# viniciusvidal2/slam-sensor-fusion

Measured on AMD Instinct MI355X. Metric: scans_per_s_200k_scan_vs_10M_map, higher is better.
Workload: dtype f32 points / f64 accumulation

## Files before the change

### include/slamfusion.h

```cpp
#ifndef SLAMFUSION_H
#define SLAMFUSION_H
#include <stdint.h>

#ifdef __cplusplus
extern "C" {
#endif

#define SF_VERSION 210

typedef enum {
    SF_OK = 0,
    SF_ERR_INVALID = -1,
    SF_ERR_HIP = -2,
    SF_ERR_NOMEM = -3,
    SF_ERR_STATE = -4,
    SF_ERR_OVERFLOW = -5,
    SF_ERR_COMM = -6
} sf_status;

typedef struct sf_ctx sf_ctx;
typedef struct sf_cloud sf_cloud;
typedef struct sf_map sf_map;
typedef struct sf_icp sf_icp;

// ... 126 lines not shown
int sf_icp_fused_count(sf_icp *icp, int64_t *launches);
int sf_icp_fused_redone(sf_icp *icp, int64_t *redone);
int sf_icp_test_inject_barrier_timeout(sf_icp *icp);
#define SF_ORDER_AUTO 0
#define SF_ORDER_AS_GIVEN 1
#define SF_ORDER_CELL 2
int sf_icp_set_query_order(sf_icp *icp, int order);
int sf_icp_set_nn_reuse(sf_icp *icp, int on);
int sf_icp_set_wide_scan_points(sf_icp *icp, int64_t points);
int sf_icp_set_pipeline(sf_icp *icp, int on);
int sf_icp_set_tile_search(sf_icp *icp, int mode);
int sf_icp_tile_info(sf_icp *icp, int64_t out[12]);
int sf_icp_set_freeze(sf_icp *icp, int on);
int sf_icp_set_freeze_params(sf_icp *icp, float guard_scale, float guard_min, float guard_max, int max_tries, int from_launch);
int sf_icp_freeze_stats(sf_icp *icp, int64_t out[5]);
#define SF_ROBUST_NONE 0
#define SF_ROBUST_HUBER 1
#define SF_ROBUST_CAUCHY 2
#define SF_ROBUST_TUKEY 3
#define SF_ROBUST_GM 4
int sf_icp_set_robust_kernel(sf_icp *icp, int kind, double k);

#define SF_COV_EIG_EPS 1e-12
#define SF_COV_FEW_CORR 1
#define SF_COV_SINGULAR 2
#define SF_COV_DEGENERATE_TRANS 4
#define SF_COV_DEGENERATE_ROT 8
typedef struct {
    double info[36];
    double cov[36];
// ... 188 lines not shown
```

### slam_sensor_fusion_amd/api.py

```python
import atexit
import ctypes as C
import os
import weakref

import numpy as np

_HERE = os.path.dirname(os.path.abspath(__file__))
LIB_PATH = os.path.join(_HERE, "lib", "libslamfusion.so")

SF_ICP_REF_CPP, SF_ICP_O3D_P2P, SF_ICP_P2PLANE = 0, 1, 2
SF_VOXEL_PCL, SF_VOXEL_O3D, SF_VOXEL_PCL64 = 0, 1, 2
SF_FLAG_VOXEL_OVERFLOW = 1
SF_ICP_FLAG_FEW_CORR, SF_ICP_FLAG_SINGULAR, SF_ICP_FLAG_SHARD_STALE, SF_ICP_FLAG_BARRIER_TIMEOUT = 1, 2, 4, 8
PROF_NN, PROF_REDUCE, PROF_COLLECTIVE, PROF_SOLVE, PROF_SHARD_BUILD = 0, 1, 2, 3, 4
SF_ERR_COMM = -6
MODES = {"ref_cpp": SF_ICP_REF_CPP, "o3d_p2p": SF_ICP_O3D_P2P, "p2plane": SF_ICP_P2PLANE}
ROBUST_KINDS = {"none": 0, "huber": 1, "cauchy": 2, "tukey": 3, "gm": 4}


class SlamFusionError(RuntimeError):
    pass


class IcpResult(C.Structure):
# ... 556 lines not shown

    def tile_info(self):
        a = (C.c_int64 * 12)()
        _check(self.lib.sf_icp_tile_info(self.h, a))
        return {"on": bool(a[0]), "cells_per_tile": [a[1], a[2], a[3]], "tiles": [a[4], a[5], a[6]], "searched": a[7], "from_lds": a[8], "left_region": a[9],
                "beyond_ring_1": a[10], "tiles_too_dense": a[11]}

    def set_freeze_params(self, guard_scale=8.0, guard_min=2.0e-5, guard_max=3.0e-4, max_tries=3, from_launch=5):
        _check(self.lib.sf_icp_set_freeze_params(self.h, C.c_float(guard_scale), C.c_float(guard_min), C.c_float(guard_max), C.c_int(max_tries), C.c_int(from_launch)))

    def freeze_stats(self):
        a = (C.c_int64 * 5)()
        _check(self.lib.sf_icp_freeze_stats(self.h, a))
        return {"froze": a[0], "thawed": a[1], "failed": a[2], "active_queries": a[3], "frozen_at_end": a[4]}

    def set_query_order(self, order="auto"):
        _check(self.lib.sf_icp_set_query_order(self.h, C.c_int({"auto": 0, "as_given": 1, "cell": 2}[order])))

    def align(self, mode="ref_cpp"):
        r = IcpResult()
        _check(self.lib.sf_icp_align(self.h, C.c_int(MODES[mode]), C.byref(r)))
        return r.as_dict()

    def align_batch(self, mode="p2plane"):
        arr = (IcpResult * self.batch)()
        _check(self.lib.sf_icp_align_batch(self.h, C.c_int(MODES[mode]), arr))
        self._prev_batch, self._last_batch = getattr(self, "_last_batch", None), self.batch
        return [r.as_dict() for r in arr]

    def align_batch_async(self, mode="p2plane"):
# ... 645 lines not shown
```

### slam_sensor_fusion_amd/csrc/sf_icp.hip

```cpp
#include "sf_common.hpp"
#include "sf_nn.hpp"
#include "sf_tile.hpp"
#include "sf_order.hpp"
#include "sf_p2p.hpp"

#include <cfloat>
#include <cstdlib>
#include <cmath>
#include <vector>
#include <mutex>
#include <string>

namespace {

constexpr int BLK = 256;
constexpr int NREC_P2P = 17;
constexpr int NREC_PLANE = 30;
constexpr int REC_STRIDE = 32;

struct IcpState {
    double T[16];
    double rec[REC_STRIDE];
    double fitness, rmse, prev_fitness, prev_rmse;
    float last_error, err_pending;
// ... 1615 lines not shown
    const int fmode = A.fz[b].mode;
    if (fmode == 2) {
        const int64_t total = A.fz[b].n_active;
        for (int bx = r; (int64_t)bx * FZ_CAP < total; bx += FZ_FEW) {
            nn_red_fz_row<Q, SHARD>(g, w, A, b, bx, 2);
            __syncthreads();
        }
        return;
    }
    for (int bx = r; bx < A.nblocks; bx += FZ_FEW) {
        nn_red_fz_row<Q, SHARD>(g, w, A, b, bx, fmode);
        __syncthreads();
    }
}

template <int STRIDE, int NCOL, int NT>
__device__ __forceinline__ void reduce_columns(const double *__restrict__ part, int nrows, double *out)
{
    constexpr int NS = 8;
    static_assert(NT % 128 == 0 && NT / 128 >= 1 && NT / 128 <= NS && NCOL <= 128, "slices of 128 columns");
    __shared__ double sl[NS][128];
    const int c = threadIdx.x & 127;
    for (int sidx = threadIdx.x >> 7; sidx < NS; sidx += NT / 128) {
        double v0 = 0, v1 = 0, v2 = 0, v3 = 0;
        if (c < NCOL) {
            int r = sidx;
            for (; r + 3 * NS < nrows; r += 4 * NS) {
                const double a0 = part[(size_t)r * STRIDE + c], a1 = part[(size_t)(r + NS) * STRIDE + c];
                const double a2 = part[(size_t)(r + 2 * NS) * STRIDE + c], a3 = part[(size_t)(r + 3 * NS) * STRIDE + c];
                v0 += a0; v1 += a1; v2 += a2; v3 += a3;
// ... 84 lines not shown
        int k = 2;
        for (int a = 0; a < 6; ++a)
            for (int c = a; c < 6; ++c) rec[k++] += A[a][c];
        for (int a = 0; a < 6; ++a) rec[23 + a] += rhs[a];
        rec[29] += SD;
    }
    __syncthreads();
}

struct FreezeBufs {
    FreezeState *fz;
    const double *mom_part;
    const uint32_t *act_cnt;
    const uint16_t *act_ids;
    uint32_t *act_all;
};

template <int NT>
__device__ __forceinline__ void freeze_fold(IcpState *S, FreezeState *F, int b, const double *__restrict__ partials, int stride, int rows, const FreezeBufs &fb, double *rec)
{
    static_assert(NT >= FZ_NMOM && NT >= 64, "the moments are copied and contracted by the first threads");
    const int fmode = F->mode;
    __shared__ double mom[FZ_NMOM];
    __shared__ double D[12];
    __shared__ uint32_t act_worst;
    __shared__ uint32_t act_total;
    const int rows_live = fmode == 2 ? (int)((F->n_active + FZ_CAP - 1) / FZ_CAP) : rows;
    reduce_partials<NREC_PLANE, NT>(partials + (size_t)b * stride * REC_STRIDE, rows_live, rec);
    if (fmode == 1) {
        reduce_columns<FZ_NMOM, FZ_NMOM, NT>(fb.mom_part + (size_t)b * stride * FZ_NMOM, rows, mom);
// ... 82 lines not shown
    if (F->mode == 0 && F->launch_mode == 0 && request && !S->done && F->tries < fp.max_tries) {
        const float gd = fmaxf((float)(m1 - m0) * fp.guard_scale, fp.guard_min);
        if (gd <= fp.guard_max) { F->guard = gd; F->mode = 1; }
    }
}

__global__ __launch_bounds__(RBLK) void k_reduce_solve_fz(IcpState *__restrict__ st, const double *__restrict__ partials, int nblocks, int n_src, int K,
                                                          const ScanBox *__restrict__ boxp, FreezeBufs fb, FreezeParams fp, int request)
{
    const int b = blockIdx.x;
    IcpState *S = st + b;
    if (S->done) return;
    FreezeState *F = fb.fz + b;
    __shared__ double rec[REC_STRIDE];
    freeze_fold<RBLK>(S, F, b, partials, nblocks, nblocks, fb, rec);
    if (threadIdx.x == 0) {
        for (int c = 0; c < NREC_PLANE; ++c) S->rec[c] = rec[c];
        double To[12];
#pragma unroll
        for (int i = 0; i < 12; ++i) To[i] = S->T[i];
        const double m0 = S->motion;
        double upd[12];
        solve_plane(S, rec, n_src, K, upd);
        track_motion(S, To, boxp[b]);
        freeze_after_update(S, F, m0, S->motion, fp, request, upd);
    }
}

__global__ void k_fz_init(FreezeState *__restrict__ fz, int batch)
{
    const int b = blockIdx.x * blockDim.x + threadIdx.x;
    if (b >= batch) return;
    FreezeState *F = fz + b;
    F->mode = 0; F->tries = 0; F->froze = 0; F->thawed = 0; F->n_active = 0; F->guard = 0.0f; F->launch_mode = 0; F->motion0 = 0.0;
}

constexpr int SBLK = 256;
template <int MODE>
__global__ __launch_bounds__(SBLK) void k_reduce_only(IcpState *__restrict__ st, const double *__restrict__ partials, int nblocks, double *__restrict__ xchg,
                                                      const uint32_t *__restrict__ own_off, int qpl, FreezeBufs fb)
{
    constexpr int NREC = MODE == 2 ? NREC_PLANE : NREC_P2P;
    const int b = blockIdx.x;
    __shared__ double rec[REC_STRIDE];
    if (st[b].done) {
        if (threadIdx.x < REC_STRIDE) xchg[(size_t)b * REC_STRIDE + threadIdx.x] = 0.0;
        return;
    }
    const int rows = own_off ? (int)((own_off[b + 1] - own_off[b] + BLK * qpl - 1) / (BLK * qpl)) : nblocks;
    if (MODE == 2 && fb.fz) freeze_fold<SBLK>(st + b, fb.fz + b, b, partials, nblocks, rows, fb, rec);
    else reduce_partials<NREC, SBLK>(partials + (size_t)b * nblocks * REC_STRIDE, rows, rec);
    if (threadIdx.x < REC_STRIDE) xchg[(size_t)b * REC_STRIDE + threadIdx.x] = rec[threadIdx.x];
}

template <int MODE>
__global__ void k_solve_only(IcpState *__restrict__ st, const double *__restrict__ xchg, int n_src, int K, int batch, const ScanBox *__restrict__ boxp, float margin,
                             FreezeState *__restrict__ fz, FreezeParams fp, int request)
{
    constexpr int NREC = MODE == 2 ? NREC_PLANE : NREC_P2P;
    const int b = blockIdx.x * blockDim.x + threadIdx.x;
    if (b >= batch) return;
    IcpState *S = st + b;
    if (S->done) return;
    double rec[REC_STRIDE];
#pragma unroll
    for (int c = 0; c < REC_STRIDE; ++c) rec[c] = c < NREC ? xchg[(size_t)b * REC_STRIDE + c] : 0.0;
// ... 556 lines not shown
        int mode = -1, iters = -1, batch = -1, window = -1, ordered = -1, reuse = -1, robust_kind = -1, cov_on = -1;
        int64_t n = -1;
        const void *map = nullptr;
        uint64_t map_generation = 0, epochs = 0;
        float max_corr = 0, accept = 0, eps = 0;
        double robust_k = 0;
        double cov_prm[5] = {0, 0, 0, 0, 0};
        bool operator==(const GraphKey &o) const
        {
            return mode == o.mode && iters == o.iters && batch == o.batch && window == o.window && ordered == o.ordered && reuse == o.reuse && n == o.n && map == o.map &&
                   map_generation == o.map_generation && epochs == o.epochs && max_corr == o.max_corr && accept == o.accept && eps == o.eps &&
                   robust_kind == o.robust_kind && robust_k == o.robust_k && cov_on == o.cov_on && std::memcmp(cov_prm, o.cov_prm, sizeof(cov_prm)) == 0;
        }
    } graph_key;
    struct Lane {
        sf::DevBuf X, qcache, Xq, qkeys, qkeys2, qidx, qidx2, corr, state, d_inits, partials, fz_state, fz_part, fz_cnt, fz_ids, fz_all, qtkey, tseg, tile_stats, cov_part, cov_out;
        hipGraphExec_t graph_exec = nullptr;
        GraphKey graph_key;
        std::vector<double> inits_uploaded;
        uint32_t d_inits_epoch = 0xffffffffu;
    } other;
    struct SrcSet {
        sf::DevBuf X0, X0r, stage, d_boxes, d_box_parts, n_dev;
        int64_t n = 0, n_cap = 0, plane = 0;
        int batch = 0, nblocks = 0, nblocks_nn = 0, qpl = 1;
        bool have_source = false, n_on_device = false;
    } other_src;
    int src_set = 0;
    hipEvent_t src_used[2] = {nullptr, nullptr}, src_ready = nullptr;
    bool src_used_rec[2] = {false, false};
    bool src_ahead = false;
// ... 26 lines not shown
    std::vector<hipEvent_t> ev;
    size_t ev_used = 0;
    int64_t prof_launches = 0;
    double prof_ms = 0;
    std::vector<float> prof_each;
    std::vector<int> ev_kind;
    std::vector<float> prof_phase[SF_PROF_KINDS];
    sf::DevBuf nn_stats;
    int freeze = 1;
    FreezeParams fz_prm{8.0f, 2.0e-5f, 3.0e-4f, 3};
    int fz_from = 5;
    bool fz_from_auto = true;
    int fz_fetches = 0;
    int fz_step = 0;
    sf::DevBuf fz_state, fz_part, fz_cnt, fz_ids, fz_all;
    int64_t nn_stats_used = 0;
    static constexpr int64_t NN_STATS_CAP = 1024;
    int robust_kind = SF_ROBUST_NONE;
    double robust_k = 0.0;
    int cov_on = 0;
    CovArg cov_arg{0.0, 0.0, 0.0, 0.0, 0.0};
    sf::DevBuf cov_part, cov_out;
    bool prev_cov_ok = false;
    int tile_mode = 0;
    bool tile_on = false;
    sf::SfTiles tiles{};
    sf::DevBuf qtkey, tseg, tile_stats;
};

namespace {
// ... 357 lines not shown
void prof_collect(sf_icp *icp)
{
    for (size_t k = 0; k + 1 < icp->ev_used; k += 2) {
        float ms = 0;
        if (hipEventElapsedTime(&ms, icp->ev[k], icp->ev[k + 1]) != hipSuccess) continue;
        const int kind = k / 2 < icp->ev_kind.size() ? icp->ev_kind[k / 2] : SF_PROF_NN;
        if (kind == SF_PROF_NN) { icp->prof_ms += ms; icp->prof_launches += 1; icp->prof_each.push_back(ms); }
        else if (kind > 0 && kind < SF_PROF_KINDS) icp->prof_phase[kind].push_back(ms);
    }
    icp->ev_used = 0;
}

sf_icp::GraphKey graph_key_now(const sf_icp *icp, int mode)
{
    sf_icp::GraphKey k;
    k.mode = mode; k.iters = icp->prm.num_iters; k.batch = icp->batch; k.window = icp->map->window.kind; k.ordered = (int)icp->ordered | ((int)icp->tile_on << 1); k.reuse = (int)icp->reuse | (icp->freeze << 1) | (icp->fz_from << 3);
    k.n = (mode == SF_ICP_REF_CPP && icp->batch == 1) ? -icp->n_cap : icp->n;
    k.map = (const void *)icp->map;
    k.map_generation = icp->map->generation;
    k.robust_kind = robust_on(icp, mode) ? icp->robust_kind : SF_ROBUST_NONE; k.robust_k = robust_on(icp, mode) ? icp->robust_k : 0.0;
    k.cov_on = icp->cov_on;
    if (icp->cov_on) { const double cp[5] = {icp->cov_arg.sensor_sigma, icp->cov_arg.thr_t, icp->cov_arg.thr_r, icp->cov_arg.infl_t, icp->cov_arg.infl_r}; std::memcpy(k.cov_prm, cp, sizeof(cp)); }
    k.max_corr = icp->prm.max_corr; k.accept = icp->prm.accept; k.eps = icp->prm.eps + icp->fz_prm.guard_scale * 1.0e-3f + icp->fz_prm.guard_min + icp->fz_prm.guard_max + (float)icp->fz_prm.max_tries;
    const sf::DevBuf *bufs[] = {&icp->X0, &icp->X0r, &icp->X, &icp->Xq, &icp->qcache, &icp->corr, &icp->state, &icp->partials, &icp->d_box, &icp->d_boxes, &icp->n_dev,
                                &icp->map->pts4, &icp->map->nrm4, &icp->map->cell_start, &icp->map->d_window, &icp->fz_state, &icp->fz_part, &icp->fz_cnt, &icp->fz_ids, &icp->fz_all, &icp->tseg, &icp->tile_stats, &icp->cov_part, &icp->cov_out};
    k.epochs = (uint64_t)icp->plane;
    for (const sf::DevBuf *b : bufs) k.epochs = (k.epochs * 1000003ull + b->epoch) * 1000003ull + (uint64_t)(uintptr_t)b->p;
    return k;
}

float o3d_thr(const sf_icp *icp) { return (float)((double)icp->prm.max_corr * (double)icp->prm.max_corr); }

template <int MODE>
void launch_nn_red(sf_icp *icp, bool sharded = false, bool one_per_lane = false)
{
    sf_map *m = icp->map;
    const int nb = sharded ? (one_per_lane ? icp->own_nblocks * icp->qpl : icp->own_nblocks) : (one_per_lane ? icp->nblocks : icp->nblocks_nn);
    const dim3 grid((unsigned)((nb + 7) & ~7), (unsigned)icp->batch), blk(BLK);
    const float *x = src(icp, 0), *y = src(icp, 1), *z = src(icp, 2);
    const IcpState *st = icp->state.as<IcpState>();
// ... 59 lines not shown
{
    const int64_t queries = icp->shard ? icp->own_total : icp->n * icp->batch;
    const bool wanted = icp->freeze == 2 || (icp->freeze == 1 && queries >= FREEZE_AUTO_MIN_QUERIES);
    return mode == SF_ICP_P2PLANE && wanted && !robust_on(icp, mode) && icp->reuse && icp->qpl == SF_WIDE_QPL && icp->map->window.kind == 0 && icp->prm.num_iters > icp->fz_from + 1 &&
           icp->fz_from >= VERIFY_FROM_SEARCH;
}

int freeze_alloc(sf_icp *icp)
{
    const size_t rows = (size_t)icp->batch * (size_t)std::max(icp->nblocks_nn, icp->shard ? icp->own_nblocks : 0);
    SF_TRY(icp->fz_state.reserve(sizeof(FreezeState) * (size_t)icp->batch));
    SF_TRY(icp->fz_part.reserve(sizeof(double) * FZ_NMOM * rows));
    SF_TRY(icp->fz_cnt.reserve(sizeof(uint32_t) * rows));
    SF_TRY(icp->fz_ids.reserve(sizeof(uint16_t) * FZ_CAP * rows));
    SF_TRY(icp->fz_all.reserve(sizeof(uint32_t) * FZ_CAP * rows));
    return SF_OK;
}

FreezeBufs freeze_bufs(sf_icp *icp, bool on)
{
    FreezeBufs fb;
    fb.fz = on ? icp->fz_state.as<FreezeState>() : nullptr;
    fb.mom_part = icp->fz_part.as<double>();
    fb.act_cnt = icp->fz_cnt.as<uint32_t>();
    fb.act_ids = icp->fz_ids.as<uint16_t>();
    fb.act_all = icp->fz_all.as<uint32_t>();
    return fb;
}

void launch_nn_red_fz(sf_icp *icp, bool sharded, bool few)
{
    sf_map *m = icp->map;
    const int nb = sharded ? icp->own_nblocks : icp->nblocks_nn;
    const dim3 grid_full((unsigned)((nb + 7) & ~7), (unsigned)icp->batch), grid_few((unsigned)FZ_FEW, (unsigned)icp->batch), blk(BLK);
    ProfScope ps(icp);
    FzArgs A;
    A.X0x = src(icp, 0); A.X0y = src(icp, 1); A.X0z = src(icp, 2);
    A.n = (int)icp->n;
    A.st = icp->state.as<IcpState>();
    A.thr = o3d_thr(icp); A.xlo = icp->xlo; A.xhi = icp->xhi;
    A.partials = icp->partials.as<double>();
    A.nblocks = nb;
// ... 12 lines not shown
        if (sharded) hipLaunchKernelGGL((k_nn_red_fz_few<SF_WIDE_QPL, true>), grid_few, blk, 0, s, m->grid, m->window, A);
        else hipLaunchKernelGGL((k_nn_red_fz_few<SF_WIDE_QPL, false>), grid_few, blk, 0, s, m->grid, m->window, A);
    } else {
        if (sharded) hipLaunchKernelGGL((k_nn_red_fz<SF_WIDE_QPL, true>), grid_full, blk, 0, s, m->grid, m->window, A);
        else hipLaunchKernelGGL((k_nn_red_fz<SF_WIDE_QPL, false>), grid_full, blk, 0, s, m->grid, m->window, A);
    }
}

bool freeze_nn_now(const sf_icp *icp, int mode) { return freeze_on(icp, mode) && icp->fz_step >= icp->fz_from; }
bool freeze_solve_now(const sf_icp *icp, int mode) { return freeze_on(icp, mode) && icp->fz_step + 1 >= icp->fz_from; }
int freeze_start_pass(sf_icp *icp, int mode)
{
    icp->fz_step = 0;
    if (!freeze_on(icp, mode)) return SF_OK;
    SF_TRY(freeze_alloc(icp));
    hipLaunchKernelGGL(k_fz_init, dim3(nblk(icp->batch, 64)), dim3(64), 0, icp->ctx->stream, icp->fz_state.as<FreezeState>(), icp->batch);
    return SF_OK;
}

int launch_state_init(sf_icp *icp)
{
    hipStream_t s = icp->ctx->stream;
    const int B = icp->batch;
    InitArgs args;
    if (B <= INIT_ARGS_MAX) {
        std::memcpy(args.T, icp->inits.data(), sizeof(double) * 16 * (size_t)B);
        hipLaunchKernelGGL(k_state_init, dim3(1), dim3(64), 0, s, icp->state.as<IcpState>(), (const double *)nullptr, args, B);
        return SF_OK;
    }
    const size_t bytes = sizeof(double) * 16 * (size_t)B;
    if (icp->inits_uploaded != icp->inits || icp->d_inits_epoch != icp->d_inits.epoch) {
// ... 58 lines not shown
    hipStream_t s = icp->ctx->stream;
    IcpState *st = icp->state.as<IcpState>();
    double *part = icp->partials.as<double>();
    const int K = icp->prm.num_iters;
    const int B = icp->batch;
    const int n = (int)icp->n;
    if (mode == SF_ICP_O3D_P2P) {
        for (int k = 0; k <= K; ++k) {
            if (tile_launch(icp, k)) launch_tile_search<1>(icp, false);
            else launch_nn_red<1>(icp);
            hipLaunchKernelGGL(k_reduce_solve<1>, dim3(B), dim3(RBLK), 0, s, st, part, icp->nblocks_nn, n, k, K, icp->d_boxes.as<ScanBox>());
        }
    } else if (mode == SF_ICP_P2PLANE) {
        const bool fz = freeze_on(icp, mode);
        if (fz) {
            hipLaunchKernelGGL(k_fz_init, dim3(nblk(B, 64)), dim3(64), 0, s, icp->fz_state.as<FreezeState>(), B);
        }
        const bool wide = icp->qpl > 1 && !icp->shard;
        for (int k = 0; k < K; ++k) {
            const bool q1 = wide && k < VERIFY_FROM_SEARCH;
            if (fz && k >= icp->fz_from) launch_nn_red_fz(icp, false, k > icp->fz_from);
            else if (tile_launch(icp, k)) launch_tile_search<2>(icp, q1);
            else launch_nn_red<2>(icp, false, q1);
            if (fz && k + 1 >= icp->fz_from)
                hipLaunchKernelGGL(k_reduce_solve_fz, dim3(B), dim3(RBLK), 0, s, st, part, q1 ? icp->nblocks : icp->nblocks_nn, n, K, icp->d_boxes.as<ScanBox>(), freeze_bufs(icp, true),
                                   icp->fz_prm, (int)(k + 2 < K));
            else if (q1)
                hipLaunchKernelGGL(k_reduce_solve<2>, dim3(B), dim3(RBLK), 0, s, st, part, icp->nblocks, n, k, K, icp->d_boxes.as<ScanBox>());
            else
                hipLaunchKernelGGL(k_reduce_solve<2>, dim3(B), dim3(RBLK), 0, s, st, part, icp->nblocks_nn, n, k, K, icp->d_boxes.as<ScanBox>());
        }
    } else {
        SF_TRY(icp->X.reserve(sizeof(float) * 3 * (size_t)std::max<int64_t>(icp->plane, 1)));
        SF_TRY(icp->corr.reserve(sizeof(float4) * (size_t)std::max<int64_t>(icp->plane, 1)));
        float *Xx = soa(icp->X, icp->plane, 0), *Xy = soa(icp->X, icp->plane, 1), *Xz = soa(icp->X, icp->plane, 2);
        float4 *corr = icp->corr.as<float4>();
        const dim3 gpts((unsigned)icp->nblocks, (unsigned)B), gred((unsigned)icp->nblocks, (unsigned)B);
        const int *nl = B == 1 ? icp->n_dev.as<int>() : nullptr;
        const bool win = m->window.kind != 0;
        const float thr = icp->prm.max_corr;
// ... 444 lines not shown
    SF_CHECK(icp && out, SF_ERR_INVALID, "bad arguments");
    for (int i = 0; i < 12; ++i) out[i] = 0;
    out[0] = icp->tile_on ? 1 : 0;
    if (!icp->tile_on) return SF_OK;
    for (int a = 0; a < 3; ++a) { out[1 + a] = icp->tiles.tc[a]; out[4 + a] = icp->tiles.nt[a]; }
    if (icp->tile_stats.p) {
        SF_HIP(hipSetDevice(icp->ctx->device));
        unsigned long long h[TILE_STATS];
        SF_HIP(hipMemcpyAsync(h, icp->tile_stats.p, sizeof(h), hipMemcpyDeviceToHost, icp->ctx->stream));
        SF_HIP(hipStreamSynchronize(icp->ctx->stream));
        for (int i = 0; i < 5; ++i) out[7 + i] = (int64_t)h[i];
    }
    return SF_OK;
}

extern "C" int sf_icp_set_freeze(sf_icp *icp, int on)
{
    SF_CHECK(icp, SF_ERR_INVALID, "icp is NULL");
    SF_CHECK(on >= 0 && on <= 2, SF_ERR_INVALID, "sf_icp_set_freeze: 0 (off), 1 (auto) or 2 (always)");
    icp->freeze = on;
    return SF_OK;
}

namespace {
constexpr int FZ_FROM_DEFAULT = 5, FZ_PROBE_EVERY = 32;
void freeze_learn_schedule(sf_icp *icp)
{
    if (!icp->fz_from_auto || icp->last_fused || icp->shard || icp->last_mode != SF_ICP_P2PLANE) return;
    const int K = icp->prm.num_iters;
    if (++icp->fz_fetches >= FZ_PROBE_EVERY) { icp->fz_fetches = 0; icp->fz_from = FZ_FROM_DEFAULT; return; }
// ... 109 lines not shown

extern "C" int sf_icp_use_graph(sf_icp *icp, int on)
{
    SF_CHECK(icp, SF_ERR_INVALID, "icp is NULL");
    icp->use_graph = on != 0;
    return SF_OK;
}

namespace {
void lane_flip(sf_icp *icp)
{
    sf_icp::Lane &o = icp->other;
    raw_swap(icp->X, o.X); raw_swap(icp->qcache, o.qcache); raw_swap(icp->Xq, o.Xq); raw_swap(icp->qkeys, o.qkeys); raw_swap(icp->qkeys2, o.qkeys2);
    raw_swap(icp->qidx, o.qidx); raw_swap(icp->qidx2, o.qidx2); raw_swap(icp->corr, o.corr); raw_swap(icp->state, o.state); raw_swap(icp->d_inits, o.d_inits);
    raw_swap(icp->partials, o.partials); raw_swap(icp->fz_state, o.fz_state); raw_swap(icp->fz_part, o.fz_part); raw_swap(icp->fz_cnt, o.fz_cnt);
    raw_swap(icp->fz_ids, o.fz_ids); raw_swap(icp->fz_all, o.fz_all); raw_swap(icp->qtkey, o.qtkey); raw_swap(icp->tseg, o.tseg); raw_swap(icp->tile_stats, o.tile_stats);
    raw_swap(icp->cov_part, o.cov_part); raw_swap(icp->cov_out, o.cov_out);
    std::swap(icp->graph_exec, o.graph_exec);
    std::swap(icp->graph_key, o.graph_key);
    std::swap(icp->inits_uploaded, o.inits_uploaded);
    std::swap(icp->d_inits_epoch, o.d_inits_epoch);
    std::swap(icp->meta, icp->other_meta);
    icp->lane ^= 1;
}

int lane_reserve(sf_icp *icp)
{
    const int batch = std::max(icp->batch, 1);
    SF_TRY(icp->state.reserve(sizeof(IcpState) * (size_t)batch));
    SF_TRY(icp->d_inits.reserve(sizeof(double) * 16 * (size_t)batch));
    SF_TRY(icp->partials.reserve(sizeof(double) * (size_t)REC_STRIDE * (size_t)std::max(icp->nblocks, 1) * (size_t)batch));
// ... 58 lines not shown
        if (icp->src_used[icp->src_set] && hipEventRecord(icp->src_used[icp->src_set], ran) == hipSuccess) icp->src_used_rec[icp->src_set] = true;
        if (hipEventRecord(icp->lane_done[icp->lane], ran) != hipSuccess) return;
        icp->lane_used[icp->lane] = true;
        if (piped) { hipError_t e = hipStreamWaitEvent(main, icp->lane_done[icp->lane], 0); (void)e; }
    }
};
}

extern "C" int sf_icp_align_batch_async(sf_icp *icp, int mode)
{
    SF_TRY(check_ready(icp, mode));
    SF_CHECK(!icp->shard, SF_ERR_STATE, "a sharded alignment needs the exchange between its halves: use sf_icp_step_begin / sf_icp_step_end");
    SF_HIP(hipSetDevice(icp->ctx->device));
    icp->last_mode = mode;
    icp->last_fused = fused_eligible(icp, mode);
    SF_TRY(order_lut_prepare(icp));
    const bool beside = icp->unfetched;
    LaneScope lanes(icp, icp->pipeline != 0 && !icp->last_fused && !icp->profiling && !icp->n_on_device);
    SF_TRY(lanes.rc);
    if (!lanes.piped) SF_TRY(lane_reserve(icp));
    icp->unfetched = true;
    icp->prev_ok = lanes.piped && beside && icp->other_meta.valid;
    icp->prev_cov_ok = icp->prev_ok && icp->other_meta.cov;
    icp->meta.valid = true;
    icp->meta.cov = icp->cov_on != 0;
    icp->meta.batch = icp->batch;
    icp->meta.mode = mode;
    icp->meta.inits = icp->inits;
    hipStream_t s = icp->ctx->stream;
    if (icp->cov_on) SF_TRY(cov_alloc(icp));
// ... 235 lines not shown
    return reuse_reset(icp, own);
}

}

extern "C" int sf_icp_step_begin(sf_icp *icp, int mode, int first)
{
    SF_TRY(check_ready(icp, mode));
    SF_CHECK(mode != SF_ICP_REF_CPP, SF_ERR_INVALID, "stepping supports O3D_P2P and P2PLANE");
    SF_CHECK(first >= 0 && first <= 2, SF_ERR_INVALID, "first must be 0, 1 or 2");
    SF_CHECK(!icp->cov_on, SF_ERR_STATE, COV_DECLINE_MSG);
    SF_CHECK(first != 2 || icp->shard, SF_ERR_STATE, "resume (first = 2) is a sharded-path operation");
    SF_HIP(hipSetDevice(icp->ctx->device));
    icp->last_mode = mode;
    icp->last_fused = false;
    if (first) SF_TRY(order_lut_prepare(icp));
    if (first == 1) SF_TRY(launch_state_init(icp));
    if (icp->shard) {
        if (first) SF_TRY(shard_build(icp, first == 2));
    } else if (first) {
        SF_TRY(order_queries(icp, mode));
        SF_TRY(reuse_reset(icp, icp->n * icp->batch));
    }
    if (first) SF_TRY(freeze_start_pass(icp, mode));
    double *x = reinterpret_cast<double *>(sf_icp_exchange_ptr(icp, nullptr));
    hipStream_t s = icp->ctx->stream;
    const bool q1 = mode == SF_ICP_P2PLANE && icp->qpl > 1 && icp->fz_step < VERIFY_FROM_SEARCH;
    const int nb = icp->shard ? (q1 ? icp->own_nblocks * icp->qpl : icp->own_nblocks) : (q1 ? icp->nblocks : icp->nblocks_nn);
    const int qpl_now = q1 ? 1 : icp->qpl;
    const uint32_t *off = icp->shard ? icp->own_off.as<uint32_t>() : nullptr;
    if (mode == SF_ICP_O3D_P2P) {
        launch_nn_red<1>(icp, icp->shard);
        ProfScope ps(icp, SF_PROF_REDUCE);
        hipLaunchKernelGGL(k_reduce_only<1>, dim3(icp->batch), dim3(SBLK), 0, s, icp->state.as<IcpState>(), icp->partials.as<double>(), nb, x, off, icp->qpl, freeze_bufs(icp, false));
    } else {
        if (freeze_nn_now(icp, mode)) launch_nn_red_fz(icp, icp->shard, icp->fz_step > icp->fz_from);
        else launch_nn_red<2>(icp, icp->shard, q1);
        ProfScope ps(icp, SF_PROF_REDUCE);
        hipLaunchKernelGGL(k_reduce_only<2>, dim3(icp->batch), dim3(SBLK), 0, s, icp->state.as<IcpState>(), icp->partials.as<double>(), nb, x, off, qpl_now,
                           freeze_bufs(icp, freeze_nn_now(icp, mode)));
    }
    SF_HIP(hipGetLastError());
    return SF_OK;
}

extern "C" int sf_icp_step_end(sf_icp *icp, int mode, int last)
{
    SF_TRY(check_ready(icp, mode));
    (void)last;
    const double *x = reinterpret_cast<const double *>(sf_icp_exchange_ptr(icp, nullptr));
    hipStream_t s = icp->ctx->stream;
    const int K = icp->prm.num_iters;
    ProfScope ps(icp, SF_PROF_SOLVE);
    if (mode == SF_ICP_O3D_P2P)
        hipLaunchKernelGGL(k_solve_only<1>, dim3(nblk(icp->batch, 64)), dim3(64), 0, s, icp->state.as<IcpState>(), x, (int)icp->n, K, icp->batch, icp->d_boxes.as<ScanBox>(),
// ... 241 lines not shown
```

Baseline: 18930.

## Defer failing reuse-certificate queries to a compacted second NN search pass

After: 19310, median of 6. 1.02x the previous value.

```diff
diff --git a/include/slamfusion.h b/include/slamfusion.h
--- a/include/slamfusion.h
+++ b/include/slamfusion.h
@@ -164,6 +164,8 @@
 int sf_icp_set_freeze(sf_icp *icp, int on);
 int sf_icp_set_freeze_params(sf_icp *icp, float guard_scale, float guard_min, float guard_max, int max_tries, int from_launch);
 int sf_icp_freeze_stats(sf_icp *icp, int64_t out[5]);
+int sf_icp_set_defer_search(sf_icp *icp, int on);
+int sf_icp_defer_stats(sf_icp *icp, int64_t out[2]);
 #define SF_ROBUST_NONE 0
 #define SF_ROBUST_HUBER 1
 #define SF_ROBUST_CAUCHY 2
diff --git a/slam_sensor_fusion_amd/api.py b/slam_sensor_fusion_amd/api.py
--- a/slam_sensor_fusion_amd/api.py
+++ b/slam_sensor_fusion_amd/api.py
@@ -594,6 +594,14 @@
         _check(self.lib.sf_icp_freeze_stats(self.h, a))
         return {"froze": a[0], "thawed": a[1], "failed": a[2], "active_queries": a[3], "frozen_at_end": a[4]}
 
+    def set_defer_search(self, on=True):
+        _check(self.lib.sf_icp_set_defer_search(self.h, C.c_int(int(bool(on)))))
+
+    def defer_stats(self):
+        a = (C.c_int64 * 2)()
+        _check(self.lib.sf_icp_defer_stats(self.h, a))
+        return {"deferred_queries": a[0], "capped_waves": a[1]}
+
     def set_query_order(self, order="auto"):
         _check(self.lib.sf_icp_set_query_order(self.h, C.c_int({"auto": 0, "as_given": 1, "cell": 2}[order])))
 
diff --git a/slam_sensor_fusion_amd/csrc/sf_icp.hip b/slam_sensor_fusion_amd/csrc/sf_icp.hip
--- a/slam_sensor_fusion_amd/csrc/sf_icp.hip
+++ b/slam_sensor_fusion_amd/csrc/sf_icp.hip
@@ -1653,6 +1653,193 @@
     }
 }
 
+
+#ifndef SF_DF_WCAP
+#define SF_DF_WCAP 8
+#endif
+constexpr int DF_WCAP = SF_DF_WCAP;
+constexpr int DF_CAPPED = 255;
+static_assert((BLK / 64) * DF_WCAP <= FZ_CAP && DF_WCAP < DF_CAPPED, "a row defers fewer queries than it could list as active");
+struct DeferBufs {
+    uint8_t *cnt;
+    uint16_t *ids;
+    double *part;
+    uint32_t *stat;
+};
+
+template <int Q>
+__global__ __launch_bounds__(BLK, NN_RED_WAVES) void k_nn_red_df(SfGrid g, SfWindow w, const float *__restrict__ X0x, const float *__restrict__ X0y, const float *__restrict__ X0z,
+                                                                 int n, const IcpState *__restrict__ st, float thr, double *__restrict__ partials, int nblocks,
+                                                                 float4 *__restrict__ qcache, int64_t cache_n, uint32_t *__restrict__ stats, DeferBufs df)
+{
+    constexpr int MODE = 2;
+    constexpr int NREC = NREC_PLANE;
+    const int L = blockIdx.y * gridDim.x + blockIdx.x;
+    const int kk = L >> 3;
+    const int b = kk % (int)gridDim.y;
+    const int bx = (L & 7) * ((int)gridDim.x >> 3) + kk / (int)gridDim.y;
+    if (bx >= nblocks) return;
+    const IcpState *S = st + b;
+    if (S->done) return;
+    __shared__ sf::WaveNN nn_ws[BLK / 64];
+    __shared__ double stage[BLK / 64][32];
+    const int wv = threadIdx.x >> 6, lane = threadIdx.x & 63;
+    const size_t seg = ((size_t)b * nblocks + bx) * (BLK / 64) + wv;
+    LanePair P[Q];
+    bool need[Q];
+#pragma unroll
+    for (int u = 0; u < Q; ++u) need[u] = false;
+    const bool attempted = qcache != nullptr && S->cache_live != 0 && S->n_research >= VERIFY_FROM_SEARCH;
+    bool fast = false;
+    uint32_t listed = 0;
+    if (attempted) {
+        const float m_now = (float)S->motion;
+#pragma unroll
+        for (int u = 0; u < Q; ++u) {
+            const int slot = bx * (BLK * Q) + u * BLK + (int)threadIdx.x;
+            const QueryIn q = query_in<MODE, false>(X0x, X0y, X0z, n, b, S, 0.0f, 0.0f, nullptr, qcache, cache_n, true, slot, n);
+            sf::NNHit hit, seed;
+            float4 tn;
+            need[u] = reuse_certificate(q.valid, q.qx, q.qy, q.qz, thr, m_now, q.e, q.c1, q.c2, hit, tn, seed);
+            P[u] = make_pair(q, hit, tn);
+        }
+        uint32_t failing = 0;
+#pragma unroll
+        for (int u = 0; u < Q; ++u) failing += (uint32_t)__popcll(__ballot(need[u]));
+        fast = failing <= (uint32_t)DF_WCAP;
+        listed = fast ? failing : (uint32_t)DF_CAPPED;
+    }
+    if (lane == 0) df.cnt[seg] = (uint8_t)listed;
+    if (fast && listed != 0u) {
+        uint32_t before = 0;
+#pragma unroll
+        for (int u = 0; u < Q; ++u) {
+            const unsigned long long bal = __ballot(need[u]);
+            const uint32_t rank = (uint32_t)__builtin_amdgcn_mbcnt_hi((uint32_t)(bal >> 32), __builtin_amdgcn_mbcnt_lo((uint32_t)bal, 0u));
+            if (need[u]) df.ids[seg * DF_WCAP + before + rank] = (uint16_t)(u * BLK + (int)threadIdx.x);
+            before += (uint32_t)__popcll(bal);
+        }
+    }
+    if (!fast) {
+        asm volatile("" ::: "memory");
+#pragma unroll
+        for (int u = 0; u < Q; ++u) {
+            const int slot = bx * (BLK * Q) + u * BLK + (int)threadIdx.x;
+            P[u] = nn_pair<MODE, false, false>(g, w, X0x, X0y, X0z, n, b, S, thr, 0.0f, 0.0f, nullptr, qcache, cache_n, slot, n, &nn_ws[wv], stats);
+        }
+    }
+#pragma unroll
+    for (int h = 0; h < 2; ++h) {
+        double v[16];
+#pragma unroll
+        for (int k = 0; k < 16; ++k) v[k] = 0.0;
+#pragma unroll
+        for (int u = 0; u < Q; ++u) {
+            const PairTerms t = pair_terms<MODE>(P[u]);
+            add_half<MODE>(t, h, v);
+        }
+        const double t0 = wave_reduce_16(v);
+        if ((lane & 3) == 0) stage[wv][16 * h + (lane >> 2)] = t0;
+    }
+    __syncthreads();
+    if (threadIdx.x < NREC) {
+        const int c = threadIdx.x;
+        double *dst = partials + ((size_t)b * nblocks + bx) * REC_STRIDE;
+        dst[c] = ((stage[0][c] + stage[1][c]) + stage[2][c]) + stage[3][c];
+    }
+}
+
+template <int Q>
+__global__ __launch_bounds__(BLK, 2) void k_nn_deferred(SfGrid g, SfWindow w, const float *__restrict__ X0x, const float *__restrict__ X0y, const float *__restrict__ X0z,
+                                                                   int n, const IcpState *__restrict__ st, float thr, int nblocks, float4 *__restrict__ qcache, int64_t cache_n,
+                                                                   uint32_t *__restrict__ stats, DeferBufs df)
+{
+    constexpr int MODE = 2;
+    constexpr int NW = BLK / 64;
+    const int r = (int)blockIdx.x, b = (int)blockIdx.y;
+    const IcpState *S = st + b;
+    if (S->done) return;
+    __shared__ sf::WaveNN nn_ws[NW];
+    __shared__ double fstage[NW][32];
+    __shared__ uint32_t list[BLK * DF_WCAP];
+    __shared__ uint32_t wsum[NW];
+    __shared__ uint32_t capped;
+    const int wv = threadIdx.x >> 6, lane = threadIdx.x & 63;
+    if (threadIdx.x == 0) capped = 0u;
+    __syncthreads();
+    const int my_rows = r < nblocks ? (nblocks - r + FZ_FEW - 1) / FZ_FEW : 0;
+    const int nseg = my_rows * NW;
+    double acc = 0.0;
+    uint32_t n_listed = 0;
+    for (int s0 = 0; s0 < nseg; s0 += BLK) {
+        const int sg = s0 + (int)threadIdx.x;
+        const int bx = r + (sg / NW) * FZ_FEW;
+        const size_t seg = ((size_t)b * nblocks + bx) * NW + (sg % NW);
+        uint32_t c = sg < nseg ? (uint32_t)df.cnt[seg] : 0u;
+        if (c > (uint32_t)DF_WCAP) {
+            atomicAdd(&capped, 1u);
+            c = 0u;
+        }
+        uint32_t incl = c;
+#pragma unroll
+        for (int off = 1; off < 64; off <<= 1) {
+            const uint32_t t = __shfl_up(incl, off, 64);
+            if (lane >= off) incl += t;
+        }
+        if (lane == 63) wsum[wv] = incl;
+        __syncthreads();
+        uint32_t base = 0, total = 0;
+#pragma unroll
+        for (int ww = 0; ww < NW; ++ww) {
+            if (ww < wv) base += wsum[ww];
+            total += wsum[ww];
+        }
+        const uint32_t start = base + incl - c;
+        for (uint32_t i = 0; i < c; ++i) list[start + i] = (uint32_t)bx * (uint32_t)(BLK * Q) + (uint32_t)df.ids[seg * DF_WCAP + i];
+        __syncthreads();
+        n_listed += total;
+        for (uint32_t q0 = 0; q0 < total; q0 += BLK) {
+            const uint32_t i = q0 + (uint32_t)threadIdx.x;
+            if (q0 + (uint32_t)(wv * 64) < total) {
+                const int slot = i < total ? (int)list[i] : n;
+                const LanePair A1 = nn_pair<MODE, false, false>(g, w, X0x, X0y, X0z, n, b, S, thr, 0.0f, 0.0f, nullptr, qcache, cache_n, slot, n, &nn_ws[wv], stats);
+#pragma unroll
+                for (int h = 0; h < 2; ++h) {
+                    double v[16];
+#pragma unroll
+                    for (int k = 0; k < 16; ++k) v[k] = 0.0;
+                    const PairTerms t = pair_terms<MODE>(A1);
+                    add_half<MODE>(t, h, v);
+                    const double t0 = wave_reduce_16(v);
+                    if ((lane & 3) == 0) fstage[wv][16 * h + (lane >> 2)] = t0;
+                }
+            } else if (lane < 32) {
+                fstage[wv][lane] = 0.0;
+            }
+            __syncthreads();
+            if (threadIdx.x < 32) acc += ((fstage[0][threadIdx.x] + fstage[1][threadIdx.x]) + fstage[2][threadIdx.x]) + fstage[3][threadIdx.x];
+            __syncthreads();
+        }
+    }
+    if (threadIdx.x < REC_STRIDE) df.part[((size_t)b * FZ_FEW + r) * REC_STRIDE + threadIdx.x] = threadIdx.x < NREC_PLANE ? acc : 0.0;
+    __syncthreads();
+    if (threadIdx.x == 0) {
+        if (n_listed) atomicAdd(&df.stat[0], n_listed);
+        if (capped) atomicAdd(&df.stat[1], capped);
+    }
+}
+
+__device__ __forceinline__ void add_deferred_rows(const double *__restrict__ df_part, int b, double *rec)
+{
+    if (threadIdx.x < NREC_PLANE) {
+        double v = 0.0;
+#pragma unroll
+        for (int r = 0; r < FZ_FEW; ++r) v += df_part[((size_t)b * FZ_FEW + r) * REC_STRIDE + threadIdx.x];
+        rec[threadIdx.x] += v;
+    }
+    __syncthreads();
+}
+
 template <int STRIDE, int NCOL, int NT>
 __device__ __forceinline__ void reduce_columns(const double *__restrict__ part, int nrows, double *out)
 {
@@ -1767,6 +1954,7 @@
     const uint32_t *act_cnt;
     const uint16_t *act_ids;
     uint32_t *act_all;
+    const double *df_part;
 };
 
 template <int NT>
@@ -1879,6 +2067,7 @@
     FreezeState *F = fb.fz + b;
     __shared__ double rec[REC_STRIDE];
     freeze_fold<RBLK>(S, F, b, partials, nblocks, nblocks, fb, rec);
+    if (fb.df_part) add_deferred_rows(fb.df_part, b, rec);
     if (threadIdx.x == 0) {
         for (int c = 0; c < NREC_PLANE; ++c) S->rec[c] = rec[c];
         double To[12];
@@ -1892,9 +2081,10 @@
     }
 }
 
-__global__ void k_fz_init(FreezeState *__restrict__ fz, int batch)
+__global__ void k_fz_init(FreezeState *__restrict__ fz, int batch, uint32_t *__restrict__ df_stat)
 {
     const int b = blockIdx.x * blockDim.x + threadIdx.x;
+    if (b == 0) df_stat[0] = df_stat[1] = 0u;
     if (b >= batch) return;
     FreezeState *F = fz + b;
     F->mode = 0; F->tries = 0; F->froze = 0; F->thawed = 0; F->n_active = 0; F->guard = 0.0f; F->launch_mode = 0; F->motion0 = 0.0;
@@ -1915,6 +2105,7 @@
     const int rows = own_off ? (int)((own_off[b + 1] - own_off[b] + BLK * qpl - 1) / (BLK * qpl)) : nblocks;
     if (MODE == 2 && fb.fz) freeze_fold<SBLK>(st + b, fb.fz + b, b, partials, nblocks, rows, fb, rec);
     else reduce_partials<NREC, SBLK>(partials + (size_t)b * nblocks * REC_STRIDE, rows, rec);
+    if (MODE == 2 && fb.df_part) add_deferred_rows(fb.df_part, b, rec);
     if (threadIdx.x < REC_STRIDE) xchg[(size_t)b * REC_STRIDE + threadIdx.x] = rec[threadIdx.x];
 }
 
@@ -2501,7 +2692,7 @@
         }
     } graph_key;
     struct Lane {
-        sf::DevBuf X, qcache, Xq, qkeys, qkeys2, qidx, qidx2, corr, state, d_inits, partials, fz_state, fz_part, fz_cnt, fz_ids, fz_all, qtkey, tseg, tile_stats, cov_part, cov_out;
+        sf::DevBuf X, qcache, Xq, qkeys, qkeys2, qidx, qidx2, corr, state, d_inits, partials, fz_state, fz_part, fz_cnt, fz_ids, fz_all, df_cnt, df_ids, df_part, df_stat, qtkey, tseg, tile_stats, cov_part, cov_out;
         hipGraphExec_t graph_exec = nullptr;
         GraphKey graph_key;
         std::vector<double> inits_uploaded;
@@ -2558,6 +2749,9 @@
     int fz_fetches = 0;
     int fz_step = 0;
     sf::DevBuf fz_state, fz_part, fz_cnt, fz_ids, fz_all;
+    int defer = 1;
+    sf::DevBuf df_cnt, df_ids, df_part, df_stat;
+    bool df_planned = false;
     int64_t nn_stats_used = 0;
     static constexpr int64_t NN_STATS_CAP = 1024;
     int robust_kind = SF_ROBUST_NONE;
@@ -2945,7 +3139,7 @@
 sf_icp::GraphKey graph_key_now(const sf_icp *icp, int mode)
 {
     sf_icp::GraphKey k;
-    k.mode = mode; k.iters = icp->prm.num_iters; k.batch = icp->batch; k.window = icp->map->window.kind; k.ordered = (int)icp->ordered | ((int)icp->tile_on << 1); k.reuse = (int)icp->reuse | (icp->freeze << 1) | (icp->fz_from << 3);
+    k.mode = mode; k.iters = icp->prm.num_iters; k.batch = icp->batch; k.window = icp->map->window.kind; k.ordered = (int)icp->ordered | ((int)icp->tile_on << 1); k.reuse = (int)icp->reuse | (icp->freeze << 1) | (icp->fz_from << 3) | (icp->defer << 16);
     k.n = (mode == SF_ICP_REF_CPP && icp->batch == 1) ? -icp->n_cap : icp->n;
     k.map = (const void *)icp->map;
     k.map_generation = icp->map->generation;
@@ -2954,7 +3148,7 @@
     if (icp->cov_on) { const double cp[5] = {icp->cov_arg.sensor_sigma, icp->cov_arg.thr_t, icp->cov_arg.thr_r, icp->cov_arg.infl_t, icp->cov_arg.infl_r}; std::memcpy(k.cov_prm, cp, sizeof(cp)); }
     k.max_corr = icp->prm.max_corr; k.accept = icp->prm.accept; k.eps = icp->prm.eps + icp->fz_prm.guard_scale * 1.0e-3f + icp->fz_prm.guard_min + icp->fz_prm.guard_max + (float)icp->fz_prm.max_tries;
     const sf::DevBuf *bufs[] = {&icp->X0, &icp->X0r, &icp->X, &icp->Xq, &icp->qcache, &icp->corr, &icp->state, &icp->partials, &icp->d_box, &icp->d_boxes, &icp->n_dev,
-                                &icp->map->pts4, &icp->map->nrm4, &icp->map->cell_start, &icp->map->d_window, &icp->fz_state, &icp->fz_part, &icp->fz_cnt, &icp->fz_ids, &icp->fz_all, &icp->tseg, &icp->tile_stats, &icp->cov_part, &icp->cov_out};
+                                &icp->map->pts4, &icp->map->nrm4, &icp->map->cell_start, &icp->map->d_window, &icp->fz_state, &icp->fz_part, &icp->fz_cnt, &icp->fz_ids, &icp->fz_all, &icp->df_cnt, &icp->df_ids, &icp->df_part, &icp->df_stat, &icp->tseg, &icp->tile_stats, &icp->cov_part, &icp->cov_out};
     k.epochs = (uint64_t)icp->plane;
     for (const sf::DevBuf *b : bufs) k.epochs = (k.epochs * 1000003ull + b->epoch) * 1000003ull + (uint64_t)(uintptr_t)b->p;
     return k;
@@ -3044,10 +3238,14 @@
     SF_TRY(icp->fz_cnt.reserve(sizeof(uint32_t) * rows));
     SF_TRY(icp->fz_ids.reserve(sizeof(uint16_t) * FZ_CAP * rows));
     SF_TRY(icp->fz_all.reserve(sizeof(uint32_t) * FZ_CAP * rows));
-    return SF_OK;
-}
-
-FreezeBufs freeze_bufs(sf_icp *icp, bool on)
+    SF_TRY(icp->df_cnt.reserve(sizeof(uint8_t) * (BLK / 64) * rows));
+    SF_TRY(icp->df_ids.reserve(sizeof(uint16_t) * (BLK / 64) * DF_WCAP * rows));
+    SF_TRY(icp->df_part.reserve(sizeof(double) * REC_STRIDE * FZ_FEW * (size_t)icp->batch));
+    SF_TRY(icp->df_stat.reserve(sizeof(uint32_t) * 2));
+    return SF_OK;
+}
+
+FreezeBufs freeze_bufs(sf_icp *icp, bool on, bool deferred = false)
 {
     FreezeBufs fb;
     fb.fz = on ? icp->fz_state.as<FreezeState>() : nullptr;
@@ -3055,7 +3253,45 @@
     fb.act_cnt = icp->fz_cnt.as<uint32_t>();
     fb.act_ids = icp->fz_ids.as<uint16_t>();
     fb.act_all = icp->fz_all.as<uint32_t>();
+    fb.df_part = deferred ? icp->df_part.as<double>() : nullptr;
     return fb;
+}
+
+DeferBufs defer_bufs(sf_icp *icp)
+{
+    DeferBufs d;
+    d.cnt = icp->df_cnt.as<uint8_t>();
+    d.ids = icp->df_ids.as<uint16_t>();
+    d.part = icp->df_part.as<double>();
+    d.stat = icp->df_stat.as<uint32_t>();
+    return d;
+}
+
+bool defer_now(const sf_icp *icp, int mode, int k)
+{
+    return freeze_on(icp, mode) && icp->defer != 0 && !icp->shard && k >= VERIFY_FROM_SEARCH && k + 1 == icp->fz_from;
+}
+
+bool defer_planned(const sf_icp *icp, int mode) { return defer_now(icp, mode, icp->fz_from - 1); }
+
+void launch_nn_deferred(sf_icp *icp, uint32_t *stats)
+{
+    sf_map *m = icp->map;
+    hipLaunchKernelGGL((k_nn_deferred<SF_WIDE_QPL>), dim3((unsigned)FZ_FEW, (unsigned)icp->batch), dim3(BLK), 0, icp->ctx->stream, m->grid, m->window, src(icp, 0), src(icp, 1), src(icp, 2),
+                       (int)icp->n, icp->state.as<IcpState>(), o3d_thr(icp), icp->nblocks_nn, icp->qcache.as<float4>(), icp->cache_n, stats, defer_bufs(icp));
+}
+
+void launch_nn_red_df(sf_icp *icp)
+{
+    sf_map *m = icp->map;
+    const int nb = icp->nblocks_nn;
+    const dim3 grid((unsigned)((nb + 7) & ~7), (unsigned)icp->batch), blk(BLK);
+    ProfScope ps(icp);
+    uint32_t *stats = nullptr;
+    if (icp->profiling && icp->nn_stats.p && icp->nn_stats_used < sf_icp::NN_STATS_CAP) stats = icp->nn_stats.as<uint32_t>() + 2 * NN_STATS_SHARDS * icp->nn_stats_used++;
+    hipLaunchKernelGGL((k_nn_red_df<SF_WIDE_QPL>), grid, blk, 0, icp->ctx->stream, m->grid, m->window, src(icp, 0), src(icp, 1), src(icp, 2), (int)icp->n, icp->state.as<IcpState>(),
+                       o3d_thr(icp), icp->partials.as<double>(), nb, icp->qcache.as<float4>(), icp->cache_n, stats, defer_bufs(icp));
+    launch_nn_deferred(icp, stats);
 }
 
 void launch_nn_red_fz(sf_icp *icp, bool sharded, bool few)
@@ -3098,7 +3334,7 @@
     icp->fz_step = 0;
     if (!freeze_on(icp, mode)) return SF_OK;
     SF_TRY(freeze_alloc(icp));
-    hipLaunchKernelGGL(k_fz_init, dim3(nblk(icp->batch, 64)), dim3(64), 0, icp->ctx->stream, icp->fz_state.as<FreezeState>(), icp->batch);
+    hipLaunchKernelGGL(k_fz_init, dim3(nblk(icp->batch, 64)), dim3(64), 0, icp->ctx->stream, icp->fz_state.as<FreezeState>(), icp->batch, icp->df_stat.as<uint32_t>());
     return SF_OK;
 }
 
@@ -3187,16 +3423,18 @@
     } else if (mode == SF_ICP_P2PLANE) {
         const bool fz = freeze_on(icp, mode);
         if (fz) {
-            hipLaunchKernelGGL(k_fz_init, dim3(nblk(B, 64)), dim3(64), 0, s, icp->fz_state.as<FreezeState>(), B);
+            hipLaunchKernelGGL(k_fz_init, dim3(nblk(B, 64)), dim3(64), 0, s, icp->fz_state.as<FreezeState>(), B, icp->df_stat.as<uint32_t>());
         }
         const bool wide = icp->qpl > 1 && !icp->shard;
         for (int k = 0; k < K; ++k) {
             const bool q1 = wide && k < VERIFY_FROM_SEARCH;
+            const bool df = !q1 && defer_now(icp, mode, k);
             if (fz && k >= icp->fz_from) launch_nn_red_fz(icp, false, k > icp->fz_from);
             else if (tile_launch(icp, k)) launch_tile_search<2>(icp, q1);
+            else if (df) launch_nn_red_df(icp);
             else launch_nn_red<2>(icp, false, q1);
             if (fz && k + 1 >= icp->fz_from)
-                hipLaunchKernelGGL(k_reduce_solve_fz, dim3(B), dim3(RBLK), 0, s, st, part, q1 ? icp->nblocks : icp->nblocks_nn, n, K, icp->d_boxes.as<ScanBox>(), freeze_bufs(icp, true),
+                hipLaunchKernelGGL(k_reduce_solve_fz, dim3(B), dim3(RBLK), 0, s, st, part, q1 ? icp->nblocks : icp->nblocks_nn, n, K, icp->d_boxes.as<ScanBox>(), freeze_bufs(icp, true, df),
                                    icp->fz_prm, (int)(k + 2 < K));
             else if (q1)
                 hipLaunchKernelGGL(k_reduce_solve<2>, dim3(B), dim3(RBLK), 0, s, st, part, icp->nblocks, n, k, K, icp->d_boxes.as<ScanBox>());
@@ -3671,6 +3909,26 @@
     return SF_OK;
 }
 
+extern "C" int sf_icp_set_defer_search(sf_icp *icp, int on)
+{
+    SF_CHECK(icp, SF_ERR_INVALID, "icp is NULL");
+    icp->defer = on != 0;
+    return SF_OK;
+}
+
+extern "C" int sf_icp_defer_stats(sf_icp *icp, int64_t out[2])
+{
+    SF_CHECK(icp && out, SF_ERR_INVALID, "bad arguments");
+    out[0] = out[1] = 0;
+    if (!icp->df_planned || !icp->df_stat.p) return SF_OK;
+    uint32_t h[2] = {0u, 0u};
+    SF_HIP(hipMemcpyAsync(h, icp->df_stat.p, sizeof(h), hipMemcpyDeviceToHost, icp->ctx->stream));
+    SF_HIP(hipStreamSynchronize(icp->ctx->stream));
+    out[0] = (int64_t)h[0];
+    out[1] = (int64_t)h[1];
+    return SF_OK;
+}
+
 extern "C" int sf_icp_set_freeze(sf_icp *icp, int on)
 {
     SF_CHECK(icp, SF_ERR_INVALID, "icp is NULL");
@@ -3810,7 +4068,8 @@
     raw_swap(icp->X, o.X); raw_swap(icp->qcache, o.qcache); raw_swap(icp->Xq, o.Xq); raw_swap(icp->qkeys, o.qkeys); raw_swap(icp->qkeys2, o.qkeys2);
     raw_swap(icp->qidx, o.qidx); raw_swap(icp->qidx2, o.qidx2); raw_swap(icp->corr, o.corr); raw_swap(icp->state, o.state); raw_swap(icp->d_inits, o.d_inits);
     raw_swap(icp->partials, o.partials); raw_swap(icp->fz_state, o.fz_state); raw_swap(icp->fz_part, o.fz_part); raw_swap(icp->fz_cnt, o.fz_cnt);
-    raw_swap(icp->fz_ids, o.fz_ids); raw_swap(icp->fz_all, o.fz_all); raw_swap(icp->qtkey, o.qtkey); raw_swap(icp->tseg, o.tseg); raw_swap(icp->tile_stats, o.tile_stats);
+    raw_swap(icp->fz_ids, o.fz_ids); raw_swap(icp->fz_all, o.fz_all); raw_swap(icp->df_cnt, o.df_cnt); raw_swap(icp->df_ids, o.df_ids); raw_swap(icp->df_part, o.df_part);
+    raw_swap(icp->df_stat, o.df_stat); raw_swap(icp->qtkey, o.qtkey); raw_swap(icp->tseg, o.tseg); raw_swap(icp->tile_stats, o.tile_stats);
     raw_swap(icp->cov_part, o.cov_part); raw_swap(icp->cov_out, o.cov_out);
     std::swap(icp->graph_exec, o.graph_exec);
     std::swap(icp->graph_key, o.graph_key);
@@ -3899,6 +4158,7 @@
     SF_HIP(hipSetDevice(icp->ctx->device));
     icp->last_mode = mode;
     icp->last_fused = fused_eligible(icp, mode);
+    icp->df_planned = !icp->last_fused && defer_planned(icp, mode);
     SF_TRY(order_lut_prepare(icp));
     const bool beside = icp->unfetched;
     LaneScope lanes(icp, icp->pipeline != 0 && !icp->last_fused && !icp->profiling && !icp->n_on_device);
@@ -4164,6 +4424,7 @@
     SF_HIP(hipSetDevice(icp->ctx->device));
     icp->last_mode = mode;
     icp->last_fused = false;
+    if (first) icp->df_planned = defer_planned(icp, mode);
     if (first) SF_TRY(order_lut_prepare(icp));
     if (first == 1) SF_TRY(launch_state_init(icp));
     if (icp->shard) {
@@ -4184,11 +4445,13 @@
         ProfScope ps(icp, SF_PROF_REDUCE);
         hipLaunchKernelGGL(k_reduce_only<1>, dim3(icp->batch), dim3(SBLK), 0, s, icp->state.as<IcpState>(), icp->partials.as<double>(), nb, x, off, icp->qpl, freeze_bufs(icp, false));
     } else {
+        const bool df = !q1 && defer_now(icp, mode, icp->fz_step);
         if (freeze_nn_now(icp, mode)) launch_nn_red_fz(icp, icp->shard, icp->fz_step > icp->fz_from);
+        else if (df) launch_nn_red_df(icp);
         else launch_nn_red<2>(icp, icp->shard, q1);
         ProfScope ps(icp, SF_PROF_REDUCE);
         hipLaunchKernelGGL(k_reduce_only<2>, dim3(icp->batch), dim3(SBLK), 0, s, icp->state.as<IcpState>(), icp->partials.as<double>(), nb, x, off, qpl_now,
-                           freeze_bufs(icp, freeze_nn_now(icp, mode)));
+                           freeze_bufs(icp, freeze_nn_now(icp, mode), df));
     }
     SF_HIP(hipGetLastError());
     return SF_OK;
```
